# yxgeee/OpenIBL

Measured on NVIDIA H100. Metric: images_per_sec_extraction, higher is better.
Workload: dtype f32 (bf16x3 split on wgmma, fp32 accumulate)

## Files before the change

### openibl_b200/csrc/engine.cu

```cuda
#include <stdlib.h>

#include <mutex>
#include <new>
#include <vector>

#include "common.cuh"

namespace ibl {

static thread_local std::string g_last_error;
void set_last_error(const std::string& s) { g_last_error = s; }
void tc_set_bn_override(int bn);
void tc_set_variant_override(int v);

static const ConvLayer kVgg16[13] = {
    {3, 64, true, false},    {64, 64, true, true},
    {64, 128, true, false},  {128, 128, true, true},
    {128, 256, true, false}, {256, 256, true, false}, {256, 256, true, true},
    {256, 512, true, false}, {512, 512, true, false}, {512, 512, true, true},
    {512, 512, true, false}, {512, 512, true, false}, {512, 512, false, false}
};

struct DevBuf {
  void* p = nullptr;
// ... 1329 lines not shown

int ibl_debug_gemm_tn(ibl_engine* e, const float* A, const float* B, float* C, void* stream) {
  IBL_REQUIRE(e && A && B && C, "null argument");
  DeviceGuard g(e->device);
  e->launches += 3;
  return debug_gemm_tn(A, B, C, S(stream));
}

int ibl_debug_umma_strided(ibl_engine* e, const void* A, int rows, const void* B, int s0, int group_rows,
                            int base_mode, float* D, void* stream) {
  IBL_REQUIRE(e && A && B && D, "null argument");
  DeviceGuard g(e->device);
  e->launches += 1;
  return debug_gmma_strided(A, rows, B, s0, group_rows, 8 * group_rows, base_mode, D, S(stream));
}

int ibl_debug_umma_halo_view(ibl_engine* e, const void* A, int rows, const void* B, int s0, int group_rows,
                             int half_rows, float* D, void* stream) {
  IBL_REQUIRE(e && A && B && D, "null argument");
  DeviceGuard g(e->device);
  e->launches += 1;
  return debug_gmma_strided(A, rows, B, s0, group_rows, half_rows, 0, D, S(stream));
}

int ibl_debug_wgmma_rs_halo_view(ibl_engine* e, const void* W, const void* X, int pitch, int hrows, int n, int s0,
                                 float* D, void* stream) {
  IBL_REQUIRE(e && W && X && D, "null argument");
  DeviceGuard g(e->device);
  e->launches += 1;
  return debug_wgmma_rs_halo(W, X, pitch, hrows, n, s0, D, S(stream));
}

int ibl_debug_set_conv3x3_variant(ibl_engine* e, int variant) {
  IBL_REQUIRE(e && variant >= 0 && variant <= 2, "bad argument");
  tc_set_variant_override(variant);
  return IBL_OK;
}

int ibl_debug_conv1_fused(ibl_engine* e, const float* x, int N, int H, int W, void* y_hi, void* y_lo, void* stream) {
  IBL_REQUIRE(e && x && y_hi && y_lo && N >= 1 && H >= 2 && W >= 2, "bad argument");
  if (!e->vgg_ready) { set_last_error("ibl_engine_set_vgg16 was not called"); return IBL_ERR_NOT_READY; }
  DeviceGuard g(e->device);
  e->launches += 1;
  return launch_conv1_fused_tc(x, e->w0_oihw, e->conv[0].bias, e->conv[1], N, H, W, static_cast<__nv_bfloat16*>(y_hi),
                               static_cast<__nv_bfloat16*>(y_lo), S(stream));
}

int ibl_debug_time_layer(ibl_engine* e, int layer, const float* x, int N, int H, int W, int bn_override,
                         int reps, float* ms_out) {
  IBL_REQUIRE(e && x && ms_out && layer >= -1 && layer <= 12 && reps >= 1, "bad argument");
  if (!e->vgg_ready) { set_last_error("ibl_engine_set_vgg16 was not called"); return IBL_ERR_NOT_READY; }
  DeviceGuard g(e->device);
  const bool fused1 = layer < 0;
  const ConvLayer& L = kVgg16[fused1 ? 1 : layer];
  const size_t in_e = (size_t)N * H * W * L.cin;
  const int oh = L.pool ? H / 2 : H, ow = L.pool ? W / 2 : W;
  const size_t out_e = (size_t)N * oh * ow * L.cout;
  IBL_RET(e->act[0].ensure((in_e > out_e ? in_e : out_e) * 4));
  IBL_RET(e->act[1].ensure((in_e > out_e ? in_e : out_e) * 4));
  cudaEvent_t e0, e1;
  IBL_CUDA_OK(cudaEventCreate(&e0));
  IBL_CUDA_OK(cudaEventCreate(&e1));
  __nv_bfloat16* ih = e->act[0].as<__nv_bfloat16>();
  __nv_bfloat16* oh_ = e->act[1].as<__nv_bfloat16>();
  int rc = IBL_OK;
  if (layer > 0) rc = launch_f32_to_planes(x, in_e, ih, ih + in_e, nullptr);
  tc_set_bn_override(bn_override);
// ... 26 lines not shown
```

### openibl_b200/csrc/tc_conv.cu

```cuda
#include "common.cuh"
#include "tc_common.cuh"

namespace ibl {

using namespace tc;

namespace tc {
EncodeTiledFn get_encode_tiled() {
  static const EncodeTiledFn fn = []() -> EncodeTiledFn {
    void* p = nullptr;
    cudaDriverEntryPointQueryResult qres;
    if (cudaGetDriverEntryPoint("cuTensorMapEncodeTiled", &p, cudaEnableDefault, &qres) ==
            cudaSuccess &&
        qres == cudaDriverEntryPointSuccess)
      return reinterpret_cast<EncodeTiledFn>(p);
    return nullptr;
  }();
  return fn;
}

int make_tmap(CUtensorMap* out, CUtensorMapDataType dt, int rank, const void* base,
              const uint64_t* dims, const uint64_t* strides_bytes, const uint32_t* box, int swizzle_bytes) {
  EncodeTiledFn enc = get_encode_tiled();
  if (!enc) {
// ... 134 lines not shown
#pragma unroll
        for (int j = 0; j < 8; ++j) o[j] = make_float4(v[4 * j], v[4 * j + 1], v[4 * j + 2], v[4 * j + 3]);
      } else {
        uint32_t hi[16], lo[16];
#pragma unroll
        for (int j = 0; j < 16; ++j) {
          const float x0 = v[2 * j], x1 = v[2 * j + 1];
          const __nv_bfloat16 h0b = __float2bfloat16_rn(x0), h1b = __float2bfloat16_rn(x1);
          __nv_bfloat162 hh(h0b, h1b);
          hi[j] = *reinterpret_cast<uint32_t*>(&hh);
          lo[j] = pack_bf16x2(x0 - __bfloat162float(h0b), x1 - __bfloat162float(h1b));
        }
        uint4* oh4 = reinterpret_cast<uint4*>(a.y_hi + off);
        uint4* ol4 = reinterpret_cast<uint4*>(a.y_lo + off);
#pragma unroll
        for (int j = 0; j < 4; ++j) {
          oh4[j] = make_uint4(hi[4 * j], hi[4 * j + 1], hi[4 * j + 2], hi[4 * j + 3]);
          ol4[j] = make_uint4(lo[4 * j], lo[4 * j + 1], lo[4 * j + 2], lo[4 * j + 3]);
        }
      }
    }
  }
  if (a.ssq && valid && !a.pool) a.ssq[(long long)nt * a.ssq_stride + pix] = ssq_acc;
}

constexpr int TC_BM = 128;
constexpr int TC_BK = 64;
constexpr int TC_A_BYTES = TC_BM * TC_BK * 2;

constexpr int TC_HALO_W = 10, TC_HALO_H = 18;
constexpr int TC_HALO_ROWS = TC_HALO_W * TC_HALO_H;
constexpr int TC_HALO_PLANE = 23 * 1024;

constexpr int TC_WIDE_PX = 256;
constexpr int TC_WIDE_HALO_PLANE = 41 * 1024;

template <int BN, int STAGES, bool HALO = false, int NA = 0, int WTW = 0>
struct ConvTcSmem {
  static constexpr int THREADS = HALO ? 384 : 160;
  static constexpr int CONSUMERS = HALO ? 2 : 1;
  static constexpr int B_BYTES = BN * TC_BK * 2;
  static constexpr int STAGE_BYTES = HALO ? 2 * B_BYTES : 2 * TC_A_BYTES + 2 * B_BYTES;
  static constexpr int HALO_PLANE = WTW ? TC_WIDE_HALO_PLANE : TC_HALO_PLANE;
  static constexpr int A_RING = HALO ? NA * 2 * HALO_PLANE : 0;
  static constexpr int STG = WTW ? 0 : CONSUMERS * ACC_STG_BYTES;
  static constexpr int BYTES = A_RING + STAGES * STAGE_BYTES + STG + 1024  + 256 ;
};

struct AccWide {
  float d[2][64];
};

__device__ __forceinline__ float wide_pick(bool swap, float a, float b) { return swap ? b : a; }

__device__ __forceinline__ void wide_transpose4(uint32_t (&x)[4][2], int j) {
#pragma unroll
  for (int bit = 0; bit < 2; ++bit) {
    const bool mine = ((j >> bit) & 1) != 0;
#pragma unroll
    for (int p0 = 0; p0 < 4; ++p0) {
      if (p0 & (1 << bit)) continue;
      const int p1 = p0 | (1 << bit);
#pragma unroll
      for (int h = 0; h < 2; ++h) {
        const uint32_t got = __shfl_xor_sync(0xffffffffu, mine ? x[p0][h] : x[p1][h], 4 << bit);
        if (mine) x[p0][h] = got; else x[p1][h] = got;
      }
    }
  }
}

__device__ __forceinline__ void conv_wide_epilogue(const ConvTcArgs& a, const AccWide& acc, int img, int h0, int w0,
                                                   int nt) {
  constexpr int NV = 2, TH = 16;
  const int t = threadIdx.x & 127, w = t >> 5, lane = t & 31, g = lane >> 2, q = lane & 3, j = g & 3;
  const bool sw = (g >> 2) != 0;
  const int c = nt * 64 + 16 * w + 2 * g;
  const int cst = nt * 64 + 16 * w + 8 * (g >> 2);
  const float b0 = __ldg(a.bias + c), b1 = __ldg(a.bias + c + 1);
  auto activate = [&](float& v0, float& v1) {
    v0 += b0; v1 += b1;
    if (a.relu) { v0 = fmaxf(v0, 0.f); v1 = fmaxf(v1, 0.f); }
  };
  auto pack = [&](float v0, float v1, uint32_t (&x)[2]) {
    if (a.y_f32) {
      x[0] = __float_as_uint(v0); x[1] = __float_as_uint(v1);
    } else {
      const __nv_bfloat16 h0b = __float2bfloat16_rn(v0), h1b = __float2bfloat16_rn(v1);
      __nv_bfloat162 hh(h0b, h1b);
      x[0] = *reinterpret_cast<uint32_t*>(&hh);
      x[1] = pack_bf16x2(v0 - __bfloat162float(h0b), v1 - __bfloat162float(h1b));
    }
  };
  auto store = [&](const uint32_t (&x)[4][2], bool valid, long long pix) {
    if (!valid) return;
    const long long off = pix * a.cout + cst;
    if (a.y_f32) {
      float4* o = reinterpret_cast<float4*>(a.y_f32 + off);
      o[0] = make_float4(__uint_as_float(x[0][0]), __uint_as_float(x[0][1]), __uint_as_float(x[1][0]), __uint_as_float(x[1][1]));
      o[1] = make_float4(__uint_as_float(x[2][0]), __uint_as_float(x[2][1]), __uint_as_float(x[3][0]), __uint_as_float(x[3][1]));
    } else {
      *reinterpret_cast<uint4*>(a.y_hi + off) = make_uint4(x[0][0], x[1][0], x[2][0], x[3][0]);
      *reinterpret_cast<uint4*>(a.y_lo + off) = make_uint4(x[0][1], x[1][1], x[2][1], x[3][1]);
    }
  };
  if (a.pool) {
    const int OH = a.H >> 1, OW = a.W >> 1;
    const int ow = (w0 >> 1) + q;
#pragma unroll
    for (int v = 0; v < NV; ++v)
#pragma unroll
      for (int m = 0; m < TH / 8; ++m) {
        uint32_t x[4][2];
#pragma unroll
        for (int p = 0; p < 4; ++p) {
          const float* r0 = &acc.d[v][4 * (2 * (4 * m + p))];
          const float* r1 = r0 + 4;
          const float e0 = fmaxf(fmaxf(r0[0], r0[1]), fmaxf(r1[0], r1[1]));
          const float e1 = fmaxf(fmaxf(r0[2], r0[3]), fmaxf(r1[2], r1[3]));
          float v0 = wide_pick(sw, e0, e1), v1 = wide_pick(sw, e1, e0);
          activate(v0, v1);
          pack(v0, v1, x[p]);
        }
        wide_transpose4(x, j);
        const int oh = (h0 >> 1) + 4 * m + j, owv = ow + 4 * v;
        store(x, oh < OH && owv < OW && img < a.N, ((long long)img * OH + oh) * OW + owv);
      }
    return;
  }
#pragma unroll
  for (int v = 0; v < NV; ++v)
#pragma unroll
    for (int b = 0; b < TH / 2; ++b) {
      uint32_t x[4][2];
      float sq[4];
#pragma unroll
      for (int p = 0; p < 4; ++p) {
        const float* r = &acc.d[v][4 * (2 * b + (p >> 1)) + (p & 1)];
        const float e0 = r[0], e1 = r[2];
        float v0 = wide_pick(sw, e0, e1), v1 = wide_pick(sw, e1, e0);
        activate(v0, v1);
        sq[p] = fmaf(v1, v1, v0 * v0);
        pack(v0, v1, x[p]);
      }
      wide_transpose4(x, j);
      const int h = h0 + 2 * b + (j >> 1), wc = w0 + 8 * v + 2 * q + (j & 1);
      const bool valid = h < a.H && wc < a.W && img < a.N;
      const long long pix = ((long long)img * a.H + h) * a.W + wc;
      store(x, valid, pix);
      if (a.ssq) {
        float mine = 0.f;
#pragma unroll
        for (int p = 0; p < 4; ++p) {
          float s2 = sq[p];
          s2 += __shfl_xor_sync(0xffffffffu, s2, 4);
          s2 += __shfl_xor_sync(0xffffffffu, s2, 8);
          s2 += __shfl_xor_sync(0xffffffffu, s2, 16);
          if (p == j) mine = s2;
        }
        if (valid && g < 4) a.ssq[(long long)(nt * 4 + w) * a.ssq_stride + pix] = mine;
      }
    }
}

template <int BN, int STAGES, bool HALO, int NA, int WTW = 0>
__global__ void __launch_bounds__(ConvTcSmem<BN, STAGES, HALO, NA, WTW>::THREADS, 1)
conv3x3_tc_kernel(const __grid_constant__ CUtensorMap tm_xhi, const __grid_constant__ CUtensorMap tm_xlo,
                  const __grid_constant__ CUtensorMap tm_whi, const __grid_constant__ CUtensorMap tm_wlo,
                  const ConvTcArgs a) {
  extern __shared__ __align__(1024) uint8_t smem_raw[];
  uint8_t* smem = reinterpret_cast<uint8_t*>((reinterpret_cast<uintptr_t>(smem_raw) + 1023) & ~uintptr_t(1023));
  using L = ConvTcSmem<BN, STAGES, HALO, NA, WTW>;
  constexpr int HALO_PLANE = L::HALO_PLANE;
  constexpr int HALO_STAGE = 2 * HALO_PLANE;
  constexpr int PX = WTW ? TC_WIDE_PX : TC_BM;
  constexpr int B_BYTES = L::B_BYTES;
  constexpr int STAGE_BYTES = L::STAGE_BYTES;
  constexpr int A_RING = L::A_RING;
  uint8_t* ring = smem + A_RING;
  float* stg = reinterpret_cast<float*>(ring + STAGES * STAGE_BYTES);
  uint64_t* bars = reinterpret_cast<uint64_t*>(ring + STAGES * STAGE_BYTES + L::STG);
  uint64_t* full_bar = bars;
  uint64_t* empty_bar = bars + STAGES;
  uint64_t* afull_bar = bars + 2 * STAGES;
  uint64_t* aempty_bar = afull_bar + NA;
  uint64_t* order_bar = aempty_bar + NA;

  const int warp = threadIdx.x >> 5, lane = threadIdx.x & 31;
  const int worker = (int)blockIdx.x;
  const int n_workers = (int)gridDim.x;
  const int producer_warp = HALO ? 0 : 4;
  if (warp == producer_warp && lane == 0) {
    tma_prefetch_desc(&tm_xhi);
    tma_prefetch_desc(&tm_xlo);
    tma_prefetch_desc(&tm_whi);
    tma_prefetch_desc(&tm_wlo);
    for (int i = 0; i < STAGES; ++i) {
      mbar_init(&full_bar[i], 1);
      mbar_init(&empty_bar[i], 4);
    }
    for (int i = 0; i < NA; ++i) {
      mbar_init(&afull_bar[i], 1);
      mbar_init(&aempty_bar[i], 4);
    }
    if (HALO) {
      mbar_init(&order_bar[0], 4);
      mbar_init(&order_bar[1], 4);
    }
// ... 26 lines not shown
      tma_load_3d_a(st, &tm_whi, fb, c0, n0, tap);
      tma_load_3d_a(st + B_BYTES, &tm_wlo, fb, c0, n0, tap);
    };
    int stage = 0;
    uint32_t phase = 0;
    if constexpr (HALO) {
      auto try_wait_warp = [&](uint32_t bar, uint32_t parity) -> bool {
        uint32_t ok = 0;
        if (lane == 0) {
          asm volatile(
              "{\n\t"
              ".reg .pred p;\n\t"
              "mbarrier.try_wait.parity.shared::cta.b64 p, [%1], %2;\n\t"
              "selp.u32 %0, 1, 0, p;\n\t"
              "}"
              : "=r"(ok)
              : "r"(bar), "r"(parity)
              : "memory");
        }
        return warp_uniform(ok) != 0;
      };
      int astage = 0;
      uint32_t aphase = 0;
      int tA = worker, kcA = 0, tB = worker, kcB = 0, tapB = 0;
      while (tB < a.total_tiles) {
        const uint32_t as_u = warp_uniform((uint32_t)astage);
        if (tA < a.total_tiles && try_wait_warp(aempty_a + 8 * as_u, aphase ^ 1)) {
          int img, h0, w0, nt;
          coords(tA, img, h0, w0, nt);
          img = (int)warp_uniform((uint32_t)img); h0 = (int)warp_uniform((uint32_t)h0);
          w0 = (int)warp_uniform((uint32_t)w0);
          const int c0 = (int)warp_uniform((uint32_t)(kcA * TC_BK));
          const uint32_t sa = smem_a + as_u * HALO_STAGE;
          constexpr uint32_t kHaloBytes = WTW ? 2u * (WTW + 2) * (TC_WIDE_PX / WTW + 2) * 128u : 2u * TC_HALO_ROWS * 128u;
          if (elect_one()) {
            mbar_arrive_expect_tx_a(afull_a + 8 * as_u, kHaloBytes);
            tma_load_4d_a(sa, &tm_xhi, afull_a + 8 * as_u, c0, w0 - 1, h0 - 1, img);
            tma_load_4d_a(sa + HALO_PLANE, &tm_xlo, afull_a + 8 * as_u, c0, w0 - 1, h0 - 1, img);
          }
          __syncwarp();
          if (++astage == NA) { astage = 0; aphase ^= 1; }
          if (++kcA == kchunks) { kcA = 0; tA += n_workers; }
          continue;
        }
        const uint32_t st_u = warp_uniform((uint32_t)stage);
        if (try_wait_warp(empty_a + 8 * st_u, phase ^ 1)) {
          int img, h0, w0, nt;
          coords(tB, img, h0, w0, nt);
          const int n0 = (int)warp_uniform((uint32_t)(nt * BN));
          const int c0 = (int)warp_uniform((uint32_t)(kcB * TC_BK));
          const int tap = (int)warp_uniform((uint32_t)tapB);
          const uint32_t st = ring_a + st_u * STAGE_BYTES;
          if (elect_one()) {
            mbar_arrive_expect_tx_a(full_a + 8 * st_u, STAGE_BYTES);
            load_w(st, full_a + 8 * st_u, c0, n0, tap);
          }
          __syncwarp();
          if (++stage == STAGES) { stage = 0; phase ^= 1; }
          if (++tapB == 9) { tapB = 0; if (++kcB == kchunks) { kcB = 0; tB += n_workers; } }
        }
      }
    } else
    for (int tile = worker; tile < a.total_tiles; tile += n_workers) {
      int img, h0, w0, nt;
      coords(tile, img, h0, w0, nt);
      img = (int)warp_uniform((uint32_t)img); h0 = (int)warp_uniform((uint32_t)h0);
      w0 = (int)warp_uniform((uint32_t)w0);
      const int n0 = (int)warp_uniform((uint32_t)(nt * BN));
      for (int kit = 0; kit < kiters; ++kit) {
        const int tap = (int)warp_uniform((uint32_t)(kit / kchunks));
        const int c0 = (int)warp_uniform((uint32_t)((kit - tap * kchunks) * TC_BK));
        const int kh = tap / 3 - 1, kw = tap % 3 - 1;
        const uint32_t st_u = warp_uniform((uint32_t)stage);
        mbar_wait_warp_a(empty_a + 8 * st_u, phase ^ 1);
        const uint32_t st = smem_a + st_u * STAGE_BYTES;
        if (elect_one()) {
          const uint32_t fb = full_a + 8 * st_u;
          mbar_arrive_expect_tx_a(fb, STAGE_BYTES);
          tma_load_4d_a(st, &tm_xhi, fb, c0, w0 + kw, h0 + kh, img);
          tma_load_4d_a(st + TC_A_BYTES, &tm_xlo, fb, c0, w0 + kw, h0 + kh, img);
          load_w(st + 2 * TC_A_BYTES, fb, c0, n0, tap);
        }
        __syncwarp();
        if (++stage == STAGES) { stage = 0; phase ^= 1; }
      }
    }
  } else if (!HALO || warp >= 4) {
    const uint32_t smem_a = smem_u32(smem);
    const uint32_t ring_a = smem_a + A_RING;
    auto release_w = [&](int st) {
      if (lane == 0) mbar_arrive(&empty_bar[st]);
    };
    if constexpr (WTW != 0) {
    setmaxnreg_inc<232>();
    static_assert(WTW == 16, "the wide tiles are 16x16 patches");
    constexpr int NV = 2;
    const int cw = warp / 4 - 1;
    const int wq = (threadIdx.x >> 5) & 3, jl = lane & 7, hl = (lane >> 3) & 1;
    const int wrow = 16 * wq + 2 * jl + (hl ^ (jl >> 2));
    const uint32_t halo_w = (uint32_t)WTW + 2;
    const uint64_t halo_desc = ((uint64_t)1 << 16) | ((uint64_t)((halo_w * 128) >> 4) << 32) | ((uint64_t)1 << 62);
    for (int i = cw; worker + i * n_workers < a.total_tiles; i += 2) {
      int img, h0, w0, nt;
      coords(worker + i * n_workers, img, h0, w0, nt);
      int astage = (i * kchunks) % NA, stage = (i * kiters) % STAGES;
      uint32_t aphase = (uint32_t)((i * kchunks) / NA) & 1u, phase = (uint32_t)((i * kiters) / STAGES) & 1u;
      if (i > 0) mbar_wait(&order_bar[cw], (uint32_t)((i - 1) >> 1) & 1u);
      AccWide acc;
      int prev = -1, prev_a = -1, kc = 0, tap = 0;
      uint32_t f[2][2][4];
      for (int kit = 0; kit < kiters; ++kit) {
        if (tap == 0) mbar_wait(&afull_bar[astage], aphase);
        mbar_wait(&full_bar[stage], phase);
        const uint32_t sb = ring_a + stage * STAGE_BYTES;
        ldsm_a_sw128(f[0][0], sb, wrow, 0);
        ldsm_a_sw128(f[0][1], sb + B_BYTES, wrow, 0);
        const uint32_t ha = smem_a + astage * HALO_STAGE;
        const uint32_t toff = ((uint32_t)(tap / 3) * halo_w + (uint32_t)(tap % 3)) * 128u;
        const uint64_t x_hi = halo_desc | (uint64_t)(((ha + toff) >> 4) & 0x3fffu);
        const uint64_t x_lo = halo_desc | (uint64_t)(((ha + HALO_PLANE + toff) >> 4) & 0x3fffu);
        const uint32_t acc0 = (kc > 0 || tap > 0) ? 1u : 0u;
#pragma unroll
        for (int k = 0; k < TC_BK / 16; ++k) {
          const uint32_t(&fh)[4] = f[k & 1][0];
          const uint32_t(&fl)[4] = f[k & 1][1];
          const uint64_t ko = (uint64_t)(k * 2);
          wgmma_fence();
#pragma unroll
          for (int v = 0; v < NV; ++v) WgmmaRS<256 / NV>::mma(acc.d[v], fh, x_lo + 64 * v + ko, (acc0 | k) ? 1u : 0u);
#pragma unroll
          for (int v = 0; v < NV; ++v) WgmmaRS<256 / NV>::mma(acc.d[v], fl, x_hi + 64 * v + ko, 1u);
#pragma unroll
          for (int v = 0; v < NV; ++v) WgmmaRS<256 / NV>::mma(acc.d[v], fh, x_hi + 64 * v + ko, 1u);
          wgmma_commit();
          if (k == 3 && kc == kchunks - 1 && tap == 8 && lane == 0) mbar_arrive(&order_bar[cw ^ 1]);
          wgmma_wait<1>();
          if (k == 0) {
            if (prev >= 0) release_w(prev);
            if (prev_a >= 0) {
              if (lane == 0) mbar_arrive(&aempty_bar[prev_a]);
              prev_a = -1;
            }
          }
          if (k + 1 < TC_BK / 16) {
            ldsm_a_sw128(f[(k + 1) & 1][0], sb, wrow, k + 1);
            ldsm_a_sw128(f[(k + 1) & 1][1], sb + B_BYTES, wrow, k + 1);
          }
        }
        prev = stage;
        if (++stage == STAGES) { stage = 0; phase ^= 1; }
        if (++tap == 9) {
          tap = 0;
          ++kc;
          prev_a = astage;
          if (++astage == NA) { astage = 0; aphase ^= 1; }
        }
      }
      wgmma_wait<0>();
#pragma unroll
      for (int v = 0; v < NV; ++v)
#pragma unroll
        for (int e = 0; e < 128 / NV; ++e) asm volatile("" : "+f"(acc.d[v][e])::"memory");
      release_w(prev);
      if (lane == 0) mbar_arrive(&aempty_bar[prev_a]);
      conv_wide_epilogue(a, acc, img, h0, w0, nt);
    }
    } else if constexpr (HALO) {
    setmaxnreg_inc<232>();
    const int cw = warp / 4 - 1;
    const int bar = 1 + cw;
    float* my_stg = stg + cw * (ACC_STG_BYTES / 4);
    const int m = threadIdx.x & 127;
    const int r = TW == 16 ? (m >> 3) & 7 : m >> 3;
    const int c = TW == 16 ? ((m >> 6) << 3) | (m & 7) : m & 7;
    const uint32_t halo_w = (uint32_t)TW + 2;
    const uint64_t halo_desc = ((uint64_t)1 << 16) | ((uint64_t)((halo_w * 128) >> 4) << 32) | ((uint64_t)1 << 62);
    const uint64_t a_half = (TW == 16 ? 8u : 8u * halo_w) * 128u / 16u;
    for (int i = cw; worker + i * n_workers < a.total_tiles; i += 2) {
      int img, h0, w0, nt;
      coords(worker + i * n_workers, img, h0, w0, nt);
      int astage = (i * kchunks) % NA, stage = (i * kiters) % STAGES;
      uint32_t aphase = (uint32_t)((i * kchunks) / NA) & 1u, phase = (uint32_t)((i * kiters) / STAGES) & 1u;
      if (i > 0) mbar_wait(&order_bar[cw], (uint32_t)((i - 1) >> 1) & 1u);
      Acc128<BN> acc;
      int prev = -1, prev_a = -1;
      for (int kc = 0; kc < kchunks; ++kc) {
        mbar_wait(&afull_bar[astage], aphase);
        const uint32_t ha = smem_a + astage * HALO_STAGE;
        for (int tap = 0; tap < 9; ++tap) {
          mbar_wait(&full_bar[stage], phase);
          const uint32_t toff = ((uint32_t)(tap / 3) * halo_w + (uint32_t)(tap % 3)) * 128u;
          const uint64_t a_hi = halo_desc | (uint64_t)(((ha + toff) >> 4) & 0x3fffu);
          const uint64_t a_lo = halo_desc | (uint64_t)(((ha + TC_HALO_PLANE + toff) >> 4) & 0x3fffu);
          const uint32_t sb = ring_a + stage * STAGE_BYTES;
          const uint64_t b_hi = gmma_desc_kmajor_sw128(sb), b_lo = gmma_desc_kmajor_sw128(sb + B_BYTES);
// ... 74 lines not shown
  static DeviceOnce attr_done;
  if (!attr_done.done()) {
    IBL_CUDA_OK(cudaFuncSetAttribute(conv3x3_tc_kernel<BN, STAGES, HALO, NA, WTW>,
                                     cudaFuncAttributeMaxDynamicSharedMemorySize, smem));
    attr_done.mark();
  }
  const int sms = device_sm_count();
  const int grid = a.total_tiles < sms ? a.total_tiles : sms;
  conv3x3_tc_kernel<BN, STAGES, HALO, NA, WTW>
      <<<grid, ConvTcSmem<BN, STAGES, HALO, NA, WTW>::THREADS, smem, s>>>(xhi, xlo, whi, wlo, a);
  IBL_CUDA_OK(cudaGetLastError());
  return IBL_OK;
}

static int g_tc_bn_override = 0;
void tc_set_bn_override(int bn) { g_tc_bn_override = bn; }
static int g_tc_variant_override = 0;
void tc_set_variant_override(int v) { g_tc_variant_override = v; }

int launch_conv3x3_tc(const __nv_bfloat16* x_hi, const __nv_bfloat16* x_lo, const ConvParams& p,
                      int N, int H, int W, int cin, int cout, bool relu, bool pool,
                      __nv_bfloat16* y_hi, __nv_bfloat16* y_lo, float* y_f32, cudaStream_t s, float* ssq,
                      int* ssq_parts) {
  IBL_REQUIRE(cin % 64 == 0 && cout % 64 == 0, "tensor-core conv needs Cin%64==0 and Cout%64==0");
  IBL_REQUIRE(p.w_hi && p.w_lo, "tensor-core conv: weights were not re-laid-out");
  IBL_REQUIRE(H >= 1 && W >= 1 && N >= 1, "empty conv input");
  ConvTcArgs a{};
  a.N = N; a.H = H; a.W = W; a.cin = cin; a.cout = cout;
  auto waste = [&](int tw, int px) {
    int th = px / tw;
    return (long long)cdiv(W, tw) * tw * cdiv(H, th) * th;
  };
  const int tw128 = (waste(16, 128) <= waste(8, 128)) ? 16 : 8;
  constexpr int tw256 = 16;
  bool wide = waste(tw256, 256) <= waste(tw128, 128);
  if (g_tc_bn_override) wide = false;
  if (g_tc_variant_override) wide = g_tc_variant_override == 2;
  const int TW = wide ? tw256 : tw128, TH = (wide ? TC_WIDE_PX : TC_BM) / TW;
  a.tw_log2 = TW == 16 ? 4 : 3;
  a.tiles_w = cdiv(W, TW);
  a.tiles_h = cdiv(H, TH);
  int bn = wide ? 64 : cout % 128 == 0 ? 128 : 64;
  if (!wide && g_tc_bn_override && cout % g_tc_bn_override == 0 && (g_tc_bn_override == 64 || g_tc_bn_override == 128))
    bn = g_tc_bn_override;
  const bool halo = wide || bn == 128;
  a.n_tiles = cout / bn;
  a.total_tiles = (int)((long long)N * a.tiles_h * a.tiles_w * a.n_tiles);
  a.relu = relu; a.pool = pool;
  a.bias = p.bias; a.y_hi = y_hi; a.y_lo = y_lo; a.y_f32 = y_f32;
  a.ssq = pool ? nullptr : ssq;
  a.ssq_stride = (long long)N * H * W;
  if (ssq_parts) *ssq_parts = wide ? cout / 16 : a.n_tiles;

  CUtensorMap m_xhi, m_xlo, m_whi, m_wlo;
  {
    uint64_t dims[4] = {(uint64_t)cin, (uint64_t)W, (uint64_t)H, (uint64_t)N};
    uint64_t str[3] = {(uint64_t)cin * 2, (uint64_t)W * cin * 2, (uint64_t)H * W * cin * 2};
    uint32_t box[4] = {64, (uint32_t)(halo ? TW + 2 : TW), (uint32_t)(halo ? TH + 2 : TH), 1};
    IBL_RET(make_tmap(&m_xhi, CU_TENSOR_MAP_DATA_TYPE_BFLOAT16, 4, x_hi, dims, str, box));
    IBL_RET(make_tmap(&m_xlo, CU_TENSOR_MAP_DATA_TYPE_BFLOAT16, 4, x_lo, dims, str, box));
  }
  {
    uint64_t dims[3] = {(uint64_t)cin, (uint64_t)cout, 9};
    uint64_t str[2] = {(uint64_t)cin * 2, (uint64_t)cout * cin * 2};
    uint32_t box[3] = {64, (uint32_t)bn, 1};
    IBL_RET(make_tmap(&m_whi, CU_TENSOR_MAP_DATA_TYPE_BFLOAT16, 3, p.w_hi, dims, str, box));
    IBL_RET(make_tmap(&m_wlo, CU_TENSOR_MAP_DATA_TYPE_BFLOAT16, 3, p.w_lo, dims, str, box));
  }
  if (wide) return launch_tc_variant<64, 3, true, 2, 16>(m_xhi, m_xlo, m_whi, m_wlo, a, s);
  if (halo) return launch_tc_variant<128, 3, true, 2>(m_xhi, m_xlo, m_whi, m_wlo, a, s);
  return launch_tc_variant<64, 4>(m_xhi, m_xlo, m_whi, m_wlo, a, s);
}

struct Conv1FusedArgs {
  const float* x;
  const float* w1;
  const float* bias1;
  ConvTcArgs c2;
};

constexpr int F1_HALO_W = 18;
constexpr int F1_HALO_ROWS = F1_HALO_W * F1_HALO_W;
constexpr int F1_HALO_STAGE = 2 * TC_WIDE_HALO_PLANE;
constexpr int F1_A1_TILE = 64 * 64;
constexpr int F1_W1_PLANE = 64 * 64;
constexpr int F1_W2_STAGE = 2 * 64 * TC_BK * 2;
constexpr int F1_W2_STAGES = 3;
constexpr int F1_OFF_W2 = 2 * F1_HALO_STAGE;
constexpr int F1_OFF_W1 = F1_OFF_W2 + F1_W2_STAGES * F1_W2_STAGE;
constexpr int F1_OFF_BAR = F1_OFF_W1 + 2 * F1_W1_PLANE;
constexpr int F1_SMEM = F1_OFF_BAR + 512 + 1024;

__host__ __device__ constexpr int f1_a1_off(int g, int plane) {
  return (g < 5 ? g * 2 * F1_A1_TILE : TC_WIDE_HALO_PLANE) + plane * F1_A1_TILE;
}
static_assert(2 * F1_A1_TILE == 64 * 128, "a tile's A1 fills its own halo rows of the hi plane");
static_assert(5 * 64 < F1_HALO_ROWS && 6 * 64 >= F1_HALO_ROWS && f1_a1_off(4, 1) + F1_A1_TILE <= TC_WIDE_HALO_PLANE &&
                  F1_HALO_ROWS * 128 <= TC_WIDE_HALO_PLANE,
              "six m64 tiles cover the halo, only tile 5 reaches past halo row 319, and the halo tile fits in a plane");
static_assert(F1_HALO_STAGE % 1024 == 0 && F1_OFF_W2 % 1024 == 0 && F1_OFF_W1 % 512 == 0 && f1_a1_off(5, 1) % 512 == 0,
              "swizzle atom alignment");
static_assert(F1_SMEM <= 232448, "shared-memory budget of the fused conv1 kernel");
// ... 154 lines not shown
#pragma unroll
        for (int j = 0; j < 32; ++j) asm volatile("" : "+f"(acc[j])::"memory");
        wg_sync(bar);
#pragma unroll
        for (int hf = 0; hf < 2; ++hf) {
          const int p = 64 * g + (tl & ~31) / 2 + ((tl & 31) >> 2) + 8 * hf;
          if (p < F1_HALO_ROWS) {
            const int hl = p / F1_HALO_W, wl = p - hl * F1_HALO_W;
            const int ph = h0 - 1 + hl, pw = w0 - 1 + wl;
            const bool inside = ph >= 0 && ph < a.H && pw >= 0 && pw < a.W && img < a.N;
            uint8_t* rh = halo + p * 128 + (tl & 3) * 4;
#pragma unroll
            for (int j = 0; j < 8; ++j) {
              const int ch = 8 * j + 2 * (tl & 3);
              float x0 = fmaxf(acc[4 * j + 2 * hf] + bias1_s[ch], 0.f);
              float x1 = fmaxf(acc[4 * j + 2 * hf + 1] + bias1_s[ch + 1], 0.f);
              if (!inside) { x0 = 0.f; x1 = 0.f; }
              const __nv_bfloat16 h0b = __float2bfloat16_rn(x0), h1b = __float2bfloat16_rn(x1);
              __nv_bfloat162 hv(h0b, h1b);
              const int pos = (j ^ (p & 7)) * 16;
              *reinterpret_cast<uint32_t*>(rh + pos) = *reinterpret_cast<uint32_t*>(&hv);
              *reinterpret_cast<uint32_t*>(rh + TC_WIDE_HALO_PLANE + pos) =
                  pack_bf16x2(x0 - __bfloat162float(h0b), x1 - __bfloat162float(h1b));
            }
          }
        }
        if (step + 2 < 6) issue_c1(step + 1, acc);
      }
      fence_proxy_async();
      wg_sync(bar);
      int stage = (i * 9) % F1_W2_STAGES;
      uint32_t phase = (uint32_t)((i * 9) / F1_W2_STAGES) & 1u;
      if (i > 0) mbar_wait(&order_bar[cw], (uint32_t)((i - 1) >> 1) & 1u);
      AccWide acc;
      uint32_t fw[2][2][4];
      int prev = -1;
#pragma unroll 1
      for (int tap = 0; tap < 9; ++tap) {
        mbar_wait(&w_full[stage], phase);
        const uint32_t sb = w2a + stage * F1_W2_STAGE;
        ldsm_a_sw128(fw[0][0], sb, wrow, 0);
        ldsm_a_sw128(fw[0][1], sb + F1_W2_STAGE / 2, wrow, 0);
        const uint32_t toff = (uint32_t)((tap / 3) * F1_HALO_W + tap % 3) * 128u;
        const uint64_t x_hi = kHaloDesc | (uint64_t)(((ha + toff) >> 4) & 0x3fffu);
        const uint64_t x_lo = kHaloDesc | (uint64_t)(((ha + TC_WIDE_HALO_PLANE + toff) >> 4) & 0x3fffu);
#pragma unroll
        for (int k = 0; k < TC_BK / 16; ++k) {
          const uint32_t(&fh)[4] = fw[k & 1][0];
          const uint32_t(&fl)[4] = fw[k & 1][1];
          const uint64_t ko = (uint64_t)(k * 2);
          wgmma_fence();
#pragma unroll
          for (int v = 0; v < 2; ++v) WgmmaRS<128>::mma(acc.d[v], fh, x_lo + 64 * v + ko, (tap > 0 || k > 0) ? 1u : 0u);
#pragma unroll
          for (int v = 0; v < 2; ++v) WgmmaRS<128>::mma(acc.d[v], fl, x_hi + 64 * v + ko, 1u);
#pragma unroll
          for (int v = 0; v < 2; ++v) WgmmaRS<128>::mma(acc.d[v], fh, x_hi + 64 * v + ko, 1u);
          wgmma_commit();
          if (k == 3 && tap == 8 && lane == 0) mbar_arrive(&order_bar[cw ^ 1]);
          wgmma_wait<1>();
          if (k == 0 && prev >= 0 && lane == 0) mbar_arrive(&w_empty[prev]);
          if (k + 1 < TC_BK / 16) {
            ldsm_a_sw128(fw[(k + 1) & 1][0], sb, wrow, k + 1);
            ldsm_a_sw128(fw[(k + 1) & 1][1], sb + F1_W2_STAGE / 2, wrow, k + 1);
          }
        }
        prev = stage;
// ... 97 lines not shown
```

### openibl_b200/csrc/tc_probe.cu

```cuda
#include "common.cuh"
#include "tc_common.cuh"

namespace ibl {

using namespace tc;

__device__ __forceinline__ uint64_t probe_desc(uint32_t a_addr, uint32_t sbo, int base_mode) {
  uint64_t d = 0;
  d |= (uint64_t)((a_addr >> 4) & 0x3fffu);
  d |= (uint64_t)1 << 16;
  d |= (uint64_t)((sbo >> 4) & 0x3fffu) << 32;
  if (base_mode == 1) d |= (uint64_t)((a_addr >> 7) & 7u) << 49;
  d |= (uint64_t)1 << 62;
  return d;
}

__global__ void __launch_bounds__(128, 1)
gmma_strided_probe_kernel(const __grid_constant__ CUtensorMap tm_a, const __grid_constant__ CUtensorMap tm_b,
                          int rows, int s0, int group_rows, int half_rows, int base_mode, float* __restrict__ D) {
  extern __shared__ __align__(1024) uint8_t smem_raw[];
  uint8_t* smem = reinterpret_cast<uint8_t*>((reinterpret_cast<uintptr_t>(smem_raw) + 1023) & ~uintptr_t(1023));
  uint8_t* a_sm = smem;
  uint8_t* b_sm = smem + 32768;
  float* stg = reinterpret_cast<float*>(smem + 32768 + 8192);
// ... 75 lines not shown
    mbar_init(&bars[0], 1);
    fence_barrier_init();
    fence_proxy_async();
  }
  __syncthreads();
  if (threadIdx.x == 0) {
    mbar_arrive_expect_tx(&bars[0], 8192 + x_bytes);
    tma_load_2d(w_sm, &tm_w, &bars[0], 0, 0);
    tma_load_3d(x_sm, &tm_x, &bars[0], 0, 0, 0);
  }
  mbar_wait(&bars[0], 0);
  const int t = threadIdx.x, lane = t & 31;
  const int row = 16 * (t >> 5) + (lane & 7) + 8 * ((lane >> 3) & 1);
  const uint64_t xd = ((uint64_t)1 << 16) | ((uint64_t)(((uint32_t)pitch * 128u) >> 4) << 32) | ((uint64_t)1 << 62) |
                      (uint64_t)(((smem_u32(x_sm) + (uint32_t)s0 * 128u) >> 4) & 0x3fffu);
  float d[N / 2];
  uint32_t f[4][4];
#pragma unroll
  for (int k = 0; k < 4; ++k) ldsm_a_sw128(f[k], smem_u32(w_sm), row, k);
  wgmma_fence();
#pragma unroll
  for (int k = 0; k < 4; ++k) WgmmaRS<N>::mma(d, f[k], xd + (uint64_t)(k * 2), k > 0 ? 1u : 0u);
  wgmma_commit();
  wgmma_wait<0>();
#pragma unroll
  for (int i = 0; i < N / 2; ++i) asm volatile("" : "+f"(d[i])::"memory");
  const int r0 = 16 * (t >> 5) + (lane >> 2), c0 = 2 * (lane & 3);
#pragma unroll
  for (int i = 0; i < N / 8; ++i)
#pragma unroll
    for (int e = 0; e < 4; ++e) D[(size_t)(r0 + 8 * (e >> 1)) * N + 8 * i + c0 + (e & 1)] = d[4 * i + e];
}

int debug_wgmma_rs_halo(const void* W, const void* X, int pitch, int hrows, int n, int s0, float* D, cudaStream_t s) {
  IBL_REQUIRE(n == 64 || n == 128, "probe view: n is 64 or 128");
  IBL_REQUIRE(pitch >= 8 && pitch <= 256 && hrows >= 1 && hrows <= 256 && pitch * hrows <= 352 && s0 >= 0 &&
                  s0 + (n / 8 - 1) * pitch + 8 <= pitch * hrows,
              "probe view does not fit the halo tile");
  CUtensorMap mw, mx;
  {
    uint64_t dims[2] = {64, 64};
    uint64_t str[1] = {128};
    uint32_t box[2] = {64, 64};
    IBL_RET(make_tmap(&mw, CU_TENSOR_MAP_DATA_TYPE_BFLOAT16, 2, W, dims, str, box));
  }
  {
    uint64_t dims[3] = {64, (uint64_t)pitch, (uint64_t)hrows};
    uint64_t str[2] = {128, (uint64_t)pitch * 128};
    uint32_t box[3] = {64, (uint32_t)pitch, (uint32_t)hrows};
    IBL_RET(make_tmap(&mx, CU_TENSOR_MAP_DATA_TYPE_BFLOAT16, 3, X, dims, str, box));
  }
  const int smem = 8192 + 45056 + 1024 + 64;
  const uint32_t x_bytes = (uint32_t)pitch * (uint32_t)hrows * 128u;
  if (n == 64) {
    static DeviceOnce attr_done;
    if (!attr_done.done()) {
      IBL_CUDA_OK(cudaFuncSetAttribute(wgmma_rs_halo_probe_kernel<64>, cudaFuncAttributeMaxDynamicSharedMemorySize, smem));
      attr_done.mark();
    }
    wgmma_rs_halo_probe_kernel<64><<<1, 128, smem, s>>>(mw, mx, pitch, s0, x_bytes, D);
  } else {
    static DeviceOnce attr_done;
    if (!attr_done.done()) {
      IBL_CUDA_OK(cudaFuncSetAttribute(wgmma_rs_halo_probe_kernel<128>, cudaFuncAttributeMaxDynamicSharedMemorySize, smem));
      attr_done.mark();
    }
    wgmma_rs_halo_probe_kernel<128><<<1, 128, smem, s>>>(mw, mx, pitch, s0, x_bytes, D);
  }
  IBL_CUDA_OK(cudaGetLastError());
  return IBL_OK;
}

}
```

### openibl_b200/csrc/wgmma.cuh

```cuda
#pragma once
#include <stdint.h>

namespace ibl {
namespace tc {

template <int N, bool F16, int TA, int TB> struct Wgmma;
template <int N> struct WgmmaRS;

template <> struct Wgmma<32, false, 0, 0> {
  static __device__ __forceinline__ void mma(float (&d)[16], uint64_t a, uint64_t b, uint32_t accumulate) {
    asm volatile(
        "{\n\t.reg .pred p;\n\tsetp.ne.b32 p, %18, 0;\n\t"
        "wgmma.mma_async.sync.aligned.m64n32k16.f32.bf16.bf16 {%0, %1, %2, %3, %4, %5, %6, %7, %8, %9, %10, %11, %12, %13, %14, %15}, %16, %17, p, 1, 1, 0, 0;\n\t}"
        : "+f"(d[0]), "+f"(d[1]), "+f"(d[2]), "+f"(d[3]), "+f"(d[4]), "+f"(d[5]), "+f"(d[6]), "+f"(d[7]), "+f"(d[8]), "+f"(d[9]), "+f"(d[10]), "+f"(d[11]), "+f"(d[12]), "+f"(d[13]), "+f"(d[14]), "+f"(d[15])
        : "l"(a), "l"(b), "r"(accumulate));
  }
};

template <> struct Wgmma<64, false, 0, 0> {
  static __device__ __forceinline__ void mma(float (&d)[32], uint64_t a, uint64_t b, uint32_t accumulate) {
    asm volatile(
        "{\n\t.reg .pred p;\n\tsetp.ne.b32 p, %34, 0;\n\t"
        "wgmma.mma_async.sync.aligned.m64n64k16.f32.bf16.bf16 {%0, %1, %2, %3, %4, %5, %6, %7, %8, %9, %10, %11, %12, %13, %14, %15, %16, %17, %18, %19, %20, %21, %22, %23, %24, %25, %26, %27, %28, %29, %30, %31}, %32, %33, p, 1, 1, 0, 0;\n\t}"
        : "+f"(d[0]), "+f"(d[1]), "+f"(d[2]), "+f"(d[3]), "+f"(d[4]), "+f"(d[5]), "+f"(d[6]), "+f"(d[7]), "+f"(d[8]), "+f"(d[9]), "+f"(d[10]), "+f"(d[11]), "+f"(d[12]), "+f"(d[13]), "+f"(d[14]), "+f"(d[15]), "+f"(d[16]), "+f"(d[17]), "+f"(d[18]), "+f"(d[19]), "+f"(d[20]), "+f"(d[21]), "+f"(d[22]), "+f"(d[23]), "+f"(d[24]), "+f"(d[25]), "+f"(d[26]), "+f"(d[27]), "+f"(d[28]), "+f"(d[29]), "+f"(d[30]), "+f"(d[31])
// ... 101 lines not shown
  }
};

template <> struct Wgmma<128, true, 0, 0> {
  static __device__ __forceinline__ void mma(float (&d)[64], uint64_t a, uint64_t b, uint32_t accumulate) {
    asm volatile(
        "{\n\t.reg .pred p;\n\tsetp.ne.b32 p, %66, 0;\n\t"
        "wgmma.mma_async.sync.aligned.m64n128k16.f32.f16.f16 {%0, %1, %2, %3, %4, %5, %6, %7, %8, %9, %10, %11, %12, %13, %14, %15, %16, %17, %18, %19, %20, %21, %22, %23, %24, %25, %26, %27, %28, %29, %30, %31, %32, %33, %34, %35, %36, %37, %38, %39, %40, %41, %42, %43, %44, %45, %46, %47, %48, %49, %50, %51, %52, %53, %54, %55, %56, %57, %58, %59, %60, %61, %62, %63}, %64, %65, p, 1, 1, 0, 0;\n\t}"
        : "+f"(d[0]), "+f"(d[1]), "+f"(d[2]), "+f"(d[3]), "+f"(d[4]), "+f"(d[5]), "+f"(d[6]), "+f"(d[7]), "+f"(d[8]), "+f"(d[9]), "+f"(d[10]), "+f"(d[11]), "+f"(d[12]), "+f"(d[13]), "+f"(d[14]), "+f"(d[15]), "+f"(d[16]), "+f"(d[17]), "+f"(d[18]), "+f"(d[19]), "+f"(d[20]), "+f"(d[21]), "+f"(d[22]), "+f"(d[23]), "+f"(d[24]), "+f"(d[25]), "+f"(d[26]), "+f"(d[27]), "+f"(d[28]), "+f"(d[29]), "+f"(d[30]), "+f"(d[31]), "+f"(d[32]), "+f"(d[33]), "+f"(d[34]), "+f"(d[35]), "+f"(d[36]), "+f"(d[37]), "+f"(d[38]), "+f"(d[39]), "+f"(d[40]), "+f"(d[41]), "+f"(d[42]), "+f"(d[43]), "+f"(d[44]), "+f"(d[45]), "+f"(d[46]), "+f"(d[47]), "+f"(d[48]), "+f"(d[49]), "+f"(d[50]), "+f"(d[51]), "+f"(d[52]), "+f"(d[53]), "+f"(d[54]), "+f"(d[55]), "+f"(d[56]), "+f"(d[57]), "+f"(d[58]), "+f"(d[59]), "+f"(d[60]), "+f"(d[61]), "+f"(d[62]), "+f"(d[63])
        : "l"(a), "l"(b), "r"(accumulate));
  }
};

template <> struct WgmmaRS<64> {
  static __device__ __forceinline__ void mma(float (&d)[32], const uint32_t (&a)[4], uint64_t b, uint32_t accumulate) {
    asm volatile(
        "{\n\t.reg .pred p;\n\tsetp.ne.b32 p, %37, 0;\n\t"
        "wgmma.mma_async.sync.aligned.m64n64k16.f32.bf16.bf16 {%0, %1, %2, %3, %4, %5, %6, %7, %8, %9, %10, %11, %12, %13, %14, %15, %16, %17, %18, %19, %20, %21, %22, %23, %24, %25, %26, %27, %28, %29, %30, %31}, {%32, %33, %34, %35}, %36, p, 1, 1, 0;\n\t}"
        : "+f"(d[0]), "+f"(d[1]), "+f"(d[2]), "+f"(d[3]), "+f"(d[4]), "+f"(d[5]), "+f"(d[6]), "+f"(d[7]), "+f"(d[8]), "+f"(d[9]), "+f"(d[10]), "+f"(d[11]), "+f"(d[12]), "+f"(d[13]), "+f"(d[14]), "+f"(d[15]), "+f"(d[16]), "+f"(d[17]), "+f"(d[18]), "+f"(d[19]), "+f"(d[20]), "+f"(d[21]), "+f"(d[22]), "+f"(d[23]), "+f"(d[24]), "+f"(d[25]), "+f"(d[26]), "+f"(d[27]), "+f"(d[28]), "+f"(d[29]), "+f"(d[30]), "+f"(d[31])
        : "r"(a[0]), "r"(a[1]), "r"(a[2]), "r"(a[3]), "l"(b), "r"(accumulate));
  }
};

template <> struct WgmmaRS<128> {
  static __device__ __forceinline__ void mma(float (&d)[64], const uint32_t (&a)[4], uint64_t b, uint32_t accumulate) {
    asm volatile(
        "{\n\t.reg .pred p;\n\tsetp.ne.b32 p, %69, 0;\n\t"
        "wgmma.mma_async.sync.aligned.m64n128k16.f32.bf16.bf16 {%0, %1, %2, %3, %4, %5, %6, %7, %8, %9, %10, %11, %12, %13, %14, %15, %16, %17, %18, %19, %20, %21, %22, %23, %24, %25, %26, %27, %28, %29, %30, %31, %32, %33, %34, %35, %36, %37, %38, %39, %40, %41, %42, %43, %44, %45, %46, %47, %48, %49, %50, %51, %52, %53, %54, %55, %56, %57, %58, %59, %60, %61, %62, %63}, {%64, %65, %66, %67}, %68, p, 1, 1, 0;\n\t}"
        : "+f"(d[0]), "+f"(d[1]), "+f"(d[2]), "+f"(d[3]), "+f"(d[4]), "+f"(d[5]), "+f"(d[6]), "+f"(d[7]), "+f"(d[8]), "+f"(d[9]), "+f"(d[10]), "+f"(d[11]), "+f"(d[12]), "+f"(d[13]), "+f"(d[14]), "+f"(d[15]), "+f"(d[16]), "+f"(d[17]), "+f"(d[18]), "+f"(d[19]), "+f"(d[20]), "+f"(d[21]), "+f"(d[22]), "+f"(d[23]), "+f"(d[24]), "+f"(d[25]), "+f"(d[26]), "+f"(d[27]), "+f"(d[28]), "+f"(d[29]), "+f"(d[30]), "+f"(d[31]), "+f"(d[32]), "+f"(d[33]), "+f"(d[34]), "+f"(d[35]), "+f"(d[36]), "+f"(d[37]), "+f"(d[38]), "+f"(d[39]), "+f"(d[40]), "+f"(d[41]), "+f"(d[42]), "+f"(d[43]), "+f"(d[44]), "+f"(d[45]), "+f"(d[46]), "+f"(d[47]), "+f"(d[48]), "+f"(d[49]), "+f"(d[50]), "+f"(d[51]), "+f"(d[52]), "+f"(d[53]), "+f"(d[54]), "+f"(d[55]), "+f"(d[56]), "+f"(d[57]), "+f"(d[58]), "+f"(d[59]), "+f"(d[60]), "+f"(d[61]), "+f"(d[62]), "+f"(d[63])
        : "r"(a[0]), "r"(a[1]), "r"(a[2]), "r"(a[3]), "l"(b), "r"(accumulate));
  }
};

}
}
```

Measured before the change: 1283.

## Add 8x30 wide conv tile variant using n240 wgmma for less padding waste

Adds a new wide-tile variant for the halo 3x3 conv: an 8-wide by 30-tall pixel patch (240 pixels) computed with a single m64n240k16 register-sourced wgmma per k-step instead of two n128 ones. The dispatcher picks this variant when its padded-pixel waste is lower than the 16x16 wide tile or the 128-pixel tile, so feature maps whose sizes fit 30-row strips waste fewer tensor-core cycles on padding. The pooled epilogue is generalised to handle a partial group of pool rows. It adds another kernel instantiation and a large 120-register accumulator, and the choice rests on a waste heuristic, not on measured speed.

```diff
diff --git a/openibl_b200/csrc/engine.cu b/openibl_b200/csrc/engine.cu
--- a/openibl_b200/csrc/engine.cu
+++ b/openibl_b200/csrc/engine.cu
@@ -1385,7 +1385,7 @@
 }
 
 int ibl_debug_set_conv3x3_variant(ibl_engine* e, int variant) {
-  IBL_REQUIRE(e && variant >= 0 && variant <= 2, "bad argument");
+  IBL_REQUIRE(e && variant >= 0 && variant <= 3, "bad argument");
   tc_set_variant_override(variant);
   return IBL_OK;
 }
diff --git a/openibl_b200/csrc/tc_conv.cu b/openibl_b200/csrc/tc_conv.cu
--- a/openibl_b200/csrc/tc_conv.cu
+++ b/openibl_b200/csrc/tc_conv.cu
@@ -190,7 +190,7 @@
 constexpr int TC_HALO_ROWS = TC_HALO_W * TC_HALO_H;
 constexpr int TC_HALO_PLANE = 23 * 1024;
 
-constexpr int TC_WIDE_PX = 256;
+constexpr int tc_wide_px(int wtw) { return wtw == 8 ? 240 : 256; }
 constexpr int TC_WIDE_HALO_PLANE = 41 * 1024;
 
 template <int BN, int STAGES, bool HALO = false, int NA = 0, int WTW = 0>
@@ -205,8 +205,9 @@
   static constexpr int BYTES = A_RING + STAGES * STAGE_BYTES + STG + 1024  + 256 ;
 };
 
+template <int NV, int N>
 struct AccWide {
-  float d[2][64];
+  float d[NV][N / 2];
 };
 
 __device__ __forceinline__ float wide_pick(bool swap, float a, float b) { return swap ? b : a; }
@@ -228,9 +229,11 @@
   }
 }
 
-__device__ __forceinline__ void conv_wide_epilogue(const ConvTcArgs& a, const AccWide& acc, int img, int h0, int w0,
-                                                   int nt) {
-  constexpr int NV = 2, TH = 16;
+template <int NV, int N>
+__device__ __forceinline__ void conv_wide_epilogue(const ConvTcArgs& a, const AccWide<NV, N>& acc, int img, int h0,
+                                                   int w0, int nt) {
+  constexpr int TH = N / 8;
+  static_assert(TH % 2 == 0, "whole pool windows per patch");
   const int t = threadIdx.x & 127, w = t >> 5, lane = t & 31, g = lane >> 2, q = lane & 3, j = g & 3;
   const bool sw = (g >> 2) != 0;
   const int c = nt * 64 + 16 * w + 2 * g;
@@ -263,15 +266,20 @@
     }
   };
   if (a.pool) {
+    constexpr int NB = TH / 2;
     const int OH = a.H >> 1, OW = a.W >> 1;
     const int ow = (w0 >> 1) + q;
 #pragma unroll
     for (int v = 0; v < NV; ++v)
 #pragma unroll
-      for (int m = 0; m < TH / 8; ++m) {
+      for (int m = 0; m < (NB + 3) / 4; ++m) {
         uint32_t x[4][2];
 #pragma unroll
         for (int p = 0; p < 4; ++p) {
+          if (4 * m + p >= NB) {
+            x[p][0] = 0u; x[p][1] = 0u;
+            continue;
+          }
           const float* r0 = &acc.d[v][4 * (2 * (4 * m + p))];
           const float* r1 = r0 + 4;
           const float e0 = fmaxf(fmaxf(r0[0], r0[1]), fmaxf(r1[0], r1[1]));
@@ -282,7 +290,7 @@
         }
         wide_transpose4(x, j);
         const int oh = (h0 >> 1) + 4 * m + j, owv = ow + 4 * v;
-        store(x, oh < OH && owv < OW && img < a.N, ((long long)img * OH + oh) * OW + owv);
+        store(x, 4 * m + j < NB && oh < OH && owv < OW && img < a.N, ((long long)img * OH + oh) * OW + owv);
       }
     return;
   }
@@ -331,7 +339,7 @@
   using L = ConvTcSmem<BN, STAGES, HALO, NA, WTW>;
   constexpr int HALO_PLANE = L::HALO_PLANE;
   constexpr int HALO_STAGE = 2 * HALO_PLANE;
-  constexpr int PX = WTW ? TC_WIDE_PX : TC_BM;
+  constexpr int PX = WTW ? tc_wide_px(WTW) : TC_BM;
   constexpr int B_BYTES = L::B_BYTES;
   constexpr int STAGE_BYTES = L::STAGE_BYTES;
   constexpr int A_RING = L::A_RING;
@@ -424,7 +432,8 @@
           w0 = (int)warp_uniform((uint32_t)w0);
           const int c0 = (int)warp_uniform((uint32_t)(kcA * TC_BK));
           const uint32_t sa = smem_a + as_u * HALO_STAGE;
-          constexpr uint32_t kHaloBytes = WTW ? 2u * (WTW + 2) * (TC_WIDE_PX / WTW + 2) * 128u : 2u * TC_HALO_ROWS * 128u;
+          constexpr uint32_t kHaloBytes = WTW ? 2u * (WTW + 2) * (PX / WTW + 2) * 128u : 2u * TC_HALO_ROWS * 128u;
+          static_assert(kHaloBytes <= 2u * HALO_PLANE, "the halo tile fits its plane");
           if (elect_one()) {
             mbar_arrive_expect_tx_a(afull_a + 8 * as_u, kHaloBytes);
             tma_load_4d_a(sa, &tm_xhi, afull_a + 8 * as_u, c0, w0 - 1, h0 - 1, img);
@@ -485,8 +494,9 @@
     };
     if constexpr (WTW != 0) {
     setmaxnreg_inc<232>();
-    static_assert(WTW == 16, "the wide tiles are 16x16 patches");
-    constexpr int NV = 2;
+    static_assert(WTW == 16 || WTW == 8, "the wide tiles are 16x16 or 8x30 patches");
+    constexpr int NV = WTW == 16 ? 2 : 1;
+    constexpr int VN = PX / NV;
     const int cw = warp / 4 - 1;
     const int wq = (threadIdx.x >> 5) & 3, jl = lane & 7, hl = (lane >> 3) & 1;
     const int wrow = 16 * wq + 2 * jl + (hl ^ (jl >> 2));
@@ -498,7 +508,7 @@
       int astage = (i * kchunks) % NA, stage = (i * kiters) % STAGES;
       uint32_t aphase = (uint32_t)((i * kchunks) / NA) & 1u, phase = (uint32_t)((i * kiters) / STAGES) & 1u;
       if (i > 0) mbar_wait(&order_bar[cw], (uint32_t)((i - 1) >> 1) & 1u);
-      AccWide acc;
+      AccWide<NV, VN> acc;
       int prev = -1, prev_a = -1, kc = 0, tap = 0;
       uint32_t f[2][2][4];
       for (int kit = 0; kit < kiters; ++kit) {
@@ -519,11 +529,11 @@
           const uint64_t ko = (uint64_t)(k * 2);
           wgmma_fence();
 #pragma unroll
-          for (int v = 0; v < NV; ++v) WgmmaRS<256 / NV>::mma(acc.d[v], fh, x_lo + 64 * v + ko, (acc0 | k) ? 1u : 0u);
-#pragma unroll
-          for (int v = 0; v < NV; ++v) WgmmaRS<256 / NV>::mma(acc.d[v], fl, x_hi + 64 * v + ko, 1u);
-#pragma unroll
-          for (int v = 0; v < NV; ++v) WgmmaRS<256 / NV>::mma(acc.d[v], fh, x_hi + 64 * v + ko, 1u);
+          for (int v = 0; v < NV; ++v) WgmmaRS<VN>::mma(acc.d[v], fh, x_lo + 64 * v + ko, (acc0 | k) ? 1u : 0u);
+#pragma unroll
+          for (int v = 0; v < NV; ++v) WgmmaRS<VN>::mma(acc.d[v], fl, x_hi + 64 * v + ko, 1u);
+#pragma unroll
+          for (int v = 0; v < NV; ++v) WgmmaRS<VN>::mma(acc.d[v], fh, x_hi + 64 * v + ko, 1u);
           wgmma_commit();
           if (k == 3 && kc == kchunks - 1 && tap == 8 && lane == 0) mbar_arrive(&order_bar[cw ^ 1]);
           wgmma_wait<1>();
@@ -552,7 +562,7 @@
 #pragma unroll
       for (int v = 0; v < NV; ++v)
 #pragma unroll
-        for (int e = 0; e < 128 / NV; ++e) asm volatile("" : "+f"(acc.d[v][e])::"memory");
+        for (int e = 0; e < VN / 2; ++e) asm volatile("" : "+f"(acc.d[v][e])::"memory");
       release_w(prev);
       if (lane == 0) mbar_arrive(&aempty_bar[prev_a]);
       conv_wide_epilogue(a, acc, img, h0, w0, nt);
@@ -693,11 +703,12 @@
     return (long long)cdiv(W, tw) * tw * cdiv(H, th) * th;
   };
   const int tw128 = (waste(16, 128) <= waste(8, 128)) ? 16 : 8;
-  constexpr int tw256 = 16;
-  bool wide = waste(tw256, 256) <= waste(tw128, 128);
-  if (g_tc_bn_override) wide = false;
-  if (g_tc_variant_override) wide = g_tc_variant_override == 2;
-  const int TW = wide ? tw256 : tw128, TH = (wide ? TC_WIDE_PX : TC_BM) / TW;
+  int wtw = waste(16, 256) <= waste(tw128, 128) ? 16 : 0;
+  if (waste(8, tc_wide_px(8)) < (wtw ? waste(16, 256) : waste(tw128, 128))) wtw = 8;
+  if (g_tc_bn_override) wtw = 0;
+  if (g_tc_variant_override) wtw = g_tc_variant_override == 2 ? 16 : g_tc_variant_override == 3 ? 8 : 0;
+  const bool wide = wtw != 0;
+  const int TW = wide ? wtw : tw128, TH = (wide ? tc_wide_px(wtw) : TC_BM) / TW;
   a.tw_log2 = TW == 16 ? 4 : 3;
   a.tiles_w = cdiv(W, TW);
   a.tiles_h = cdiv(H, TH);
@@ -728,7 +739,8 @@
     IBL_RET(make_tmap(&m_whi, CU_TENSOR_MAP_DATA_TYPE_BFLOAT16, 3, p.w_hi, dims, str, box));
     IBL_RET(make_tmap(&m_wlo, CU_TENSOR_MAP_DATA_TYPE_BFLOAT16, 3, p.w_lo, dims, str, box));
   }
-  if (wide) return launch_tc_variant<64, 3, true, 2, 16>(m_xhi, m_xlo, m_whi, m_wlo, a, s);
+  if (wtw == 16) return launch_tc_variant<64, 3, true, 2, 16>(m_xhi, m_xlo, m_whi, m_wlo, a, s);
+  if (wtw == 8) return launch_tc_variant<64, 3, true, 2, 8>(m_xhi, m_xlo, m_whi, m_wlo, a, s);
   if (halo) return launch_tc_variant<128, 3, true, 2>(m_xhi, m_xlo, m_whi, m_wlo, a, s);
   return launch_tc_variant<64, 4>(m_xhi, m_xlo, m_whi, m_wlo, a, s);
 }
@@ -949,7 +961,7 @@
       int stage = (i * 9) % F1_W2_STAGES;
       uint32_t phase = (uint32_t)((i * 9) / F1_W2_STAGES) & 1u;
       if (i > 0) mbar_wait(&order_bar[cw], (uint32_t)((i - 1) >> 1) & 1u);
-      AccWide acc;
+      AccWide<2, 128> acc;
       uint32_t fw[2][2][4];
       int prev = -1;
 #pragma unroll 1
diff --git a/openibl_b200/csrc/tc_probe.cu b/openibl_b200/csrc/tc_probe.cu
--- a/openibl_b200/csrc/tc_probe.cu
+++ b/openibl_b200/csrc/tc_probe.cu
@@ -131,8 +131,21 @@
     for (int e = 0; e < 4; ++e) D[(size_t)(r0 + 8 * (e >> 1)) * N + 8 * i + c0 + (e & 1)] = d[4 * i + e];
 }
 
+template <int N>
+static int launch_rs_halo_probe(const CUtensorMap& mw, const CUtensorMap& mx, int pitch, int s0, uint32_t x_bytes,
+                                float* D, int smem, cudaStream_t s) {
+  static DeviceOnce attr_done;
+  if (!attr_done.done()) {
+    IBL_CUDA_OK(cudaFuncSetAttribute(wgmma_rs_halo_probe_kernel<N>, cudaFuncAttributeMaxDynamicSharedMemorySize, smem));
+    attr_done.mark();
+  }
+  wgmma_rs_halo_probe_kernel<N><<<1, 128, smem, s>>>(mw, mx, pitch, s0, x_bytes, D);
+  IBL_CUDA_OK(cudaGetLastError());
+  return IBL_OK;
+}
+
 int debug_wgmma_rs_halo(const void* W, const void* X, int pitch, int hrows, int n, int s0, float* D, cudaStream_t s) {
-  IBL_REQUIRE(n == 64 || n == 128, "probe view: n is 64 or 128");
+  IBL_REQUIRE(n == 64 || n == 128 || n == 240, "probe view: n is 64, 128 or 240");
   IBL_REQUIRE(pitch >= 8 && pitch <= 256 && hrows >= 1 && hrows <= 256 && pitch * hrows <= 352 && s0 >= 0 &&
                   s0 + (n / 8 - 1) * pitch + 8 <= pitch * hrows,
               "probe view does not fit the halo tile");
@@ -151,23 +164,9 @@
   }
   const int smem = 8192 + 45056 + 1024 + 64;
   const uint32_t x_bytes = (uint32_t)pitch * (uint32_t)hrows * 128u;
-  if (n == 64) {
-    static DeviceOnce attr_done;
-    if (!attr_done.done()) {
-      IBL_CUDA_OK(cudaFuncSetAttribute(wgmma_rs_halo_probe_kernel<64>, cudaFuncAttributeMaxDynamicSharedMemorySize, smem));
-      attr_done.mark();
-    }
-    wgmma_rs_halo_probe_kernel<64><<<1, 128, smem, s>>>(mw, mx, pitch, s0, x_bytes, D);
-  } else {
-    static DeviceOnce attr_done;
-    if (!attr_done.done()) {
-      IBL_CUDA_OK(cudaFuncSetAttribute(wgmma_rs_halo_probe_kernel<128>, cudaFuncAttributeMaxDynamicSharedMemorySize, smem));
-      attr_done.mark();
-    }
-    wgmma_rs_halo_probe_kernel<128><<<1, 128, smem, s>>>(mw, mx, pitch, s0, x_bytes, D);
-  }
-  IBL_CUDA_OK(cudaGetLastError());
-  return IBL_OK;
+  if (n == 64) return launch_rs_halo_probe<64>(mw, mx, pitch, s0, x_bytes, D, smem, s);
+  if (n == 128) return launch_rs_halo_probe<128>(mw, mx, pitch, s0, x_bytes, D, smem, s);
+  return launch_rs_halo_probe<240>(mw, mx, pitch, s0, x_bytes, D, smem, s);
 }
 
 }
diff --git a/openibl_b200/csrc/wgmma.cuh b/openibl_b200/csrc/wgmma.cuh
--- a/openibl_b200/csrc/wgmma.cuh
+++ b/openibl_b200/csrc/wgmma.cuh
@@ -157,5 +157,15 @@
   }
 };
 
+template <> struct WgmmaRS<240> {
+  static __device__ __forceinline__ void mma(float (&d)[120], const uint32_t (&a)[4], uint64_t b, uint32_t accumulate) {
+    asm volatile(
+        "{\n\t.reg .pred p;\n\tsetp.ne.b32 p, %125, 0;\n\t"
+        "wgmma.mma_async.sync.aligned.m64n240k16.f32.bf16.bf16 {%0, %1, %2, %3, %4, %5, %6, %7, %8, %9, %10, %11, %12, %13, %14, %15, %16, %17, %18, %19, %20, %21, %22, %23, %24, %25, %26, %27, %28, %29, %30, %31, %32, %33, %34, %35, %36, %37, %38, %39, %40, %41, %42, %43, %44, %45, %46, %47, %48, %49, %50, %51, %52, %53, %54, %55, %56, %57, %58, %59, %60, %61, %62, %63, %64, %65, %66, %67, %68, %69, %70, %71, %72, %73, %74, %75, %76, %77, %78, %79, %80, %81, %82, %83, %84, %85, %86, %87, %88, %89, %90, %91, %92, %93, %94, %95, %96, %97, %98, %99, %100, %101, %102, %103, %104, %105, %106, %107, %108, %109, %110, %111, %112, %113, %114, %115, %116, %117, %118, %119}, {%120, %121, %122, %123}, %124, p, 1, 1, 0;\n\t}"
+        : "+f"(d[0]), "+f"(d[1]), "+f"(d[2]), "+f"(d[3]), "+f"(d[4]), "+f"(d[5]), "+f"(d[6]), "+f"(d[7]), "+f"(d[8]), "+f"(d[9]), "+f"(d[10]), "+f"(d[11]), "+f"(d[12]), "+f"(d[13]), "+f"(d[14]), "+f"(d[15]), "+f"(d[16]), "+f"(d[17]), "+f"(d[18]), "+f"(d[19]), "+f"(d[20]), "+f"(d[21]), "+f"(d[22]), "+f"(d[23]), "+f"(d[24]), "+f"(d[25]), "+f"(d[26]), "+f"(d[27]), "+f"(d[28]), "+f"(d[29]), "+f"(d[30]), "+f"(d[31]), "+f"(d[32]), "+f"(d[33]), "+f"(d[34]), "+f"(d[35]), "+f"(d[36]), "+f"(d[37]), "+f"(d[38]), "+f"(d[39]), "+f"(d[40]), "+f"(d[41]), "+f"(d[42]), "+f"(d[43]), "+f"(d[44]), "+f"(d[45]), "+f"(d[46]), "+f"(d[47]), "+f"(d[48]), "+f"(d[49]), "+f"(d[50]), "+f"(d[51]), "+f"(d[52]), "+f"(d[53]), "+f"(d[54]), "+f"(d[55]), "+f"(d[56]), "+f"(d[57]), "+f"(d[58]), "+f"(d[59]), "+f"(d[60]), "+f"(d[61]), "+f"(d[62]), "+f"(d[63]), "+f"(d[64]), "+f"(d[65]), "+f"(d[66]), "+f"(d[67]), "+f"(d[68]), "+f"(d[69]), "+f"(d[70]), "+f"(d[71]), "+f"(d[72]), "+f"(d[73]), "+f"(d[74]), "+f"(d[75]), "+f"(d[76]), "+f"(d[77]), "+f"(d[78]), "+f"(d[79]), "+f"(d[80]), "+f"(d[81]), "+f"(d[82]), "+f"(d[83]), "+f"(d[84]), "+f"(d[85]), "+f"(d[86]), "+f"(d[87]), "+f"(d[88]), "+f"(d[89]), "+f"(d[90]), "+f"(d[91]), "+f"(d[92]), "+f"(d[93]), "+f"(d[94]), "+f"(d[95]), "+f"(d[96]), "+f"(d[97]), "+f"(d[98]), "+f"(d[99]), "+f"(d[100]), "+f"(d[101]), "+f"(d[102]), "+f"(d[103]), "+f"(d[104]), "+f"(d[105]), "+f"(d[106]), "+f"(d[107]), "+f"(d[108]), "+f"(d[109]), "+f"(d[110]), "+f"(d[111]), "+f"(d[112]), "+f"(d[113]), "+f"(d[114]), "+f"(d[115]), "+f"(d[116]), "+f"(d[117]), "+f"(d[118]), "+f"(d[119])
+        : "r"(a[0]), "r"(a[1]), "r"(a[2]), "r"(a[3]), "l"(b), "r"(accumulate));
+  }
+};
+
 }
 }
```

After: 1317, median of 6. 2.6% higher.
